# titoeb/RecModel

Measured on AMD Instinct MI355X. Metric: ALS user+item row-updates/sec, higher is better.
Workload: dtype f32; 1 GPU; cfg3: WMF k=128+bias, 10000000x1000000 CSR, 99990947 nnz, alpha-log confidence, gamma=0.1, zipf_a=0.0; n_items=1000000, nnz=99990947, k=128, bias=True

## Files before the change

recmodel_amd/csrc/wmf_dense.hip:

```cpp
#include "wmf_common.h"
#include "wmf_internal.h"

#include <utility>

template <int NFB, int NSPLIT, int S>
__device__ __forceinline__ void gram_body(const float* __restrict__ Y, int64_t m, int f, int ld, int bias,
                                          float* __restrict__ partial, int64_t step_lo, int64_t step_hi) {
    constexpr int NT = NFB * (NFB + 1) / 2;
    constexpr int NACC = (NT + NSPLIT - 1) / NSPLIT;
    const int lane = threadIdx.x & 63;
    const int r = lane & 15, q = lane >> 4;
    f32x4 acc[NACC];
#pragma unroll
    for (int i = 0; i < NACC; ++i) acc[i] = f32x4{0.f, 0.f, 0.f, 0.f};

    constexpr int U = 4;
    float cur[U][NFB], nxt[U][NFB];
    const int last_col = min(16 * (NFB - 1) + r, ld - 1);
    const float col_mask_last = (16 * (NFB - 1) + r < f) ? 1.f : 0.f;
    auto load_trip = [&](int64_t s0, float (&fr)[U][NFB]) {
#pragma unroll
        for (int uu = 0; uu < U; ++uu) {
            const int64_t row = min(4 * (s0 + uu) + q, m - 1);
            const float* yrow = Y + row * (int64_t)ld;
#pragma unroll
            for (int fb = 0; fb < NFB - 1; ++fb) fr[uu][fb] = yrow[16 * fb + r];
            fr[uu][NFB - 1] = yrow[last_col];
        }
    };
    if (step_lo < step_hi) load_trip(step_lo, cur);
    for (int64_t s0 = step_lo; s0 < step_hi; s0 += U) {
        if (s0 + U < step_hi) load_trip(s0 + U, nxt);
#pragma unroll
        for (int uu = 0; uu < U; ++uu) {
            const int64_t s = s0 + uu;
            const float rmask = (s < step_hi && 4 * s + q < m) ? 1.f : 0.f;
            float frag[NFB];
#pragma unroll
            for (int fb = 0; fb < NFB; ++fb) frag[fb] = cur[uu][fb] * rmask;
            frag[NFB - 1] *= col_mask_last;
            if (bias && r == 0) frag[0] = rmask;
            int t = 0;
#pragma unroll
            for (int bi = 0; bi < NFB; ++bi) {
#pragma unroll
                for (int bj = bi; bj < NFB; ++bj, ++t) {
                    if (t % NSPLIT == S) acc[t / NSPLIT] = WMF_MFMA16(frag[bi], frag[bj], acc[t / NSPLIT]);
                }
            }
        }
#pragma unroll
        for (int uu = 0; uu < U; ++uu)
#pragma unroll
            for (int fb = 0; fb < NFB; ++fb) cur[uu][fb] = nxt[uu][fb];
    }
    float* out = partial + (int64_t)blockIdx.x * NT * 256;
    int t = 0;
#pragma unroll
    for (int bi = 0; bi < NFB; ++bi) {
#pragma unroll
        for (int bj = bi; bj < NFB; ++bj, ++t) {
            if (t % NSPLIT == S) {
#pragma unroll
                for (int reg = 0; reg < 4; ++reg) out[(t * 4 + reg) * 64 + lane] = acc[t / NSPLIT][reg];
            }
        }
    }
}

typedef __bf16 gram_bf16x8 __attribute__((ext_vector_type(8)));
template <int NFB>
__device__ __forceinline__ void gram_body6(const float* __restrict__ Y, int64_t m, int f, int ld, int bias,
                                           float* __restrict__ partial, int64_t step_lo, int64_t step_hi) {
    constexpr int NT = NFB * (NFB + 1) / 2;
    const int lane = threadIdx.x;
    const int r = lane & 15, q = lane >> 4;
    f32x4 acc[NT];
#pragma unroll
    for (int i = 0; i < NT; ++i) acc[i] = f32x4{0.f, 0.f, 0.f, 0.f};
    const int last_col = min(16 * (NFB - 1) + r, ld - 1);
    const float col_mask_last = (16 * (NFB - 1) + r < f) ? 1.f : 0.f;
    const int64_t row_lo = 32 * step_lo, row_hi = m, stride = 32 * step_hi;
    float cur[8][NFB], nxt[8][NFB];
    auto load_chunk = [&](int64_t c0, float (&fr)[8][NFB]) {
#pragma unroll
        for (int j = 0; j < 8; ++j) {
            const int64_t row = min(c0 + 8 * q + j, m - 1);
            const float* yrow = Y + row * (int64_t)ld;
#pragma unroll
            for (int fb = 0; fb < NFB - 1; ++fb) fr[j][fb] = yrow[16 * fb + r];
            fr[j][NFB - 1] = yrow[last_col];
        }
    };
    if (row_lo < row_hi) load_chunk(row_lo, cur);
    for (int64_t c0 = row_lo; c0 < row_hi; c0 += stride) {
        if (c0 + stride < row_hi) load_chunk(c0 + stride, nxt);
        gram_bf16x8 hi[NFB], mid[NFB], lo[NFB];
#pragma unroll
        for (int j = 0; j < 8; ++j) {
            const float rmask = (c0 + 8 * q + j < row_hi) ? 1.f : 0.f;
#pragma unroll
            for (int fb = 0; fb < NFB; ++fb) {
                float x = cur[j][fb] * rmask;
                if (fb == NFB - 1) x *= col_mask_last;
                if (fb == 0 && bias && r == 0) x = rmask;
                const __bf16 h = (__bf16)x;
                const float r1 = x - (float)h;
                const __bf16 md = (__bf16)r1;
                hi[fb][j] = h; mid[fb][j] = md; lo[fb][j] = (__bf16)(r1 - (float)md);
            }
        }
        int t0 = 0;
#pragma unroll
        for (int bi = 0; bi < NFB; ++bi) {
#pragma unroll
            for (int bj = bi; bj < NFB; ++bj) acc[t0 + bj - bi] = __builtin_amdgcn_mfma_f32_16x16x32_bf16(lo[bi], hi[bj], acc[t0 + bj - bi], 0, 0, 0);
#pragma unroll
            for (int bj = bi; bj < NFB; ++bj) acc[t0 + bj - bi] = __builtin_amdgcn_mfma_f32_16x16x32_bf16(mid[bi], mid[bj], acc[t0 + bj - bi], 0, 0, 0);
#pragma unroll
            for (int bj = bi; bj < NFB; ++bj) acc[t0 + bj - bi] = __builtin_amdgcn_mfma_f32_16x16x32_bf16(hi[bi], lo[bj], acc[t0 + bj - bi], 0, 0, 0);
#pragma unroll
            for (int bj = bi; bj < NFB; ++bj) acc[t0 + bj - bi] = __builtin_amdgcn_mfma_f32_16x16x32_bf16(mid[bi], hi[bj], acc[t0 + bj - bi], 0, 0, 0);
#pragma unroll
            for (int bj = bi; bj < NFB; ++bj) acc[t0 + bj - bi] = __builtin_amdgcn_mfma_f32_16x16x32_bf16(hi[bi], mid[bj], acc[t0 + bj - bi], 0, 0, 0);
#pragma unroll
            for (int bj = bi; bj < NFB; ++bj) acc[t0 + bj - bi] = __builtin_amdgcn_mfma_f32_16x16x32_bf16(hi[bi], hi[bj], acc[t0 + bj - bi], 0, 0, 0);
            t0 += NFB - bi;
        }
#pragma unroll
        for (int j = 0; j < 8; ++j)
#pragma unroll
            for (int fb = 0; fb < NFB; ++fb) cur[j][fb] = nxt[j][fb];
    }
    float* out = partial + (int64_t)blockIdx.x * NT * 256;
#pragma unroll
    for (int t = 0; t < NT; ++t)
#pragma unroll
        for (int reg = 0; reg < 4; ++reg) out[(t * 4 + reg) * 64 + lane] = acc[t][reg];
}

template <int NFB>
__global__ __launch_bounds__(64) void gram6_kernel(const float* __restrict__ Y, int64_t m, int f, int ld, int bias,
                                                   float* __restrict__ partial, int64_t steps_per_wave) {
    gram_body6<NFB>(Y, m, f, ld, bias, partial, blockIdx.x, gridDim.x);
}

template <int NFB, int NSPLIT>
__global__ __launch_bounds__(NSPLIT == 1 ? 64 : 256) void gram_kernel(const float* __restrict__ Y, int64_t m, int f, int ld, int bias,
                                                  float* __restrict__ partial, int64_t steps_per_wave) {
    const int64_t nsteps = (m + 3) / 4;
    int64_t lo = (int64_t)blockIdx.x * steps_per_wave;
    int64_t hi = lo + steps_per_wave;
    if (hi > nsteps) hi = nsteps;
    if (lo > hi) lo = hi;
    if constexpr (NSPLIT == 1) {
        gram_body<NFB, 1, 0>(Y, m, f, ld, bias, partial, lo, hi);
    } else {
        switch (__builtin_amdgcn_readfirstlane(threadIdx.x >> 6)) {
            case 0: gram_body<NFB, NSPLIT, 0>(Y, m, f, ld, bias, partial, lo, hi); break;
            case 1: gram_body<NFB, NSPLIT, 1>(Y, m, f, ld, bias, partial, lo, hi); break;
            case 2: gram_body<NFB, NSPLIT, 2>(Y, m, f, ld, bias, partial, lo, hi); break;
            default: gram_body<NFB, NSPLIT, 3>(Y, m, f, ld, bias, partial, lo, hi); break;
        }
    }
}

#define WMF_GRAM_SLICES 32
__global__ __launch_bounds__(256) void gram_reduce1_kernel(const float* __restrict__ partial, int nwaves, int f, int nfb,
                                                           double* __restrict__ slices) {
    const int e = blockIdx.x * blockDim.x + threadIdx.x;
    if (e >= f * f) return;
    int i = e / f, j = e % f;
    if (i > j) { int tmp = i; i = j; j = tmp; }
    const int bi = i >> 4, bj = j >> 4, ri = i & 15, cj = j & 15;
    const int t = bi * nfb - (bi * (bi - 1)) / 2 + (bj - bi);
    const int lane = cj + 16 * (ri >> 2), reg = ri & 3;
    const int nt = nfb * (nfb + 1) / 2;
    const float* p = partial + ((int64_t)t * 4 + reg) * 64 + lane;
    const int per = (nwaves + WMF_GRAM_SLICES - 1) / WMF_GRAM_SLICES;
    const int w0 = blockIdx.y * per, w1 = min(nwaves, w0 + per);
    double s = 0.0;
    for (int w = w0; w < w1; ++w) s += (double)p[(int64_t)w * nt * 256];
    slices[(int64_t)blockIdx.y * f * f + e] = s;
}

__global__ __launch_bounds__(256) void gram_reduce2_kernel(const double* __restrict__ slices, int f, double* __restrict__ G) {
    const int e = blockIdx.x * blockDim.x + threadIdx.x;
    if (e >= f * f) return;
    double s = 0.0;
#pragma unroll 8
    for (int k = 0; k < WMF_GRAM_SLICES; ++k) s += slices[(int64_t)k * f * f + e];
    G[e] = s;
}

template <int NFB>
static int launch_gram_nfb(const float* Y, int64_t m, int f, int ld, int bias, float* partial, int nwaves,
                           hipStream_t st) {
    const int64_t nsteps = (m + 3) / 4;
    const int64_t spw = (nsteps + nwaves - 1) / nwaves;
    if constexpr (NFB >= 7 && NFB <= 9) {
        if (!(wmf_debug_flags & WMF_DBG_F32_GRAM)) {
            static const char* nm = wmf_kname("gram6_kernel<%d>", NFB);
            WMF_LAUNCH(nm, (gram6_kernel<NFB>), dim3(nwaves), dim3(64), 0, st, Y, m, f, ld, bias, partial, spw);
            return 0;
        }
    }
    if constexpr (NFB <= 9) {
        static const char* nm = wmf_kname("gram_kernel<%d, 1>", NFB);
        WMF_LAUNCH(nm, (gram_kernel<NFB, 1>), dim3(nwaves), dim3(64), 0, st, Y, m, f, ld, bias, partial, spw);
    } else {
        static const char* nm = wmf_kname("gram_kernel<%d, 4>", NFB);
        WMF_LAUNCH(nm, (gram_kernel<NFB, 4>), dim3(nwaves), dim3(256), 0, st, Y, m, f, ld, bias, partial, spw);
    }
    return 0;
}

int wmf_gram_max_waves(int f) {
    const int64_t nfb = (f + 15) / 16, nt = nfb * (nfb + 1) / 2;
    int64_t cap = ((int64_t)64 << 20) / (nt * 1024);
    if (cap > WMF_GRAM_MAX_WAVES) cap = WMF_GRAM_MAX_WAVES;
    return (int)(cap < 64 ? 64 : cap);
}

int wmf_gram_nwaves(int64_t m, int f) {
    int64_t nsteps = (m + 3) / 4;
    int64_t want = (nsteps + 31) / 32;
    if (want < 1) want = 1;
    const int cap = wmf_gram_max_waves(f);
    if (want > cap) want = cap;
    if (want > 1024) want -= want % 1024;
    return (int)want;
}

int wmf_launch_gram(const float* Y, int64_t m, int f, int ld, int bias, double* G_sum, float* partial, double* slices,
                    hipStream_t st) {
    if (m <= 0) return hipMemsetAsync(G_sum, 0, (size_t)f * f * sizeof(double), st) == hipSuccess ? 0 : -1;
    const int nfb = (f + 15) / 16;
    const int nwaves = wmf_gram_nwaves(m, f);
    switch (nfb) {
#define C(N) case N: launch_gram_nfb<N>(Y, m, f, ld, bias, partial, nwaves, st); break;
        C(1) C(2) C(3) C(4) C(5) C(6) C(7) C(8) C(9) C(10) C(11) C(12) C(13) C(14) C(15) C(16) C(17)
#undef C
        default: return -1;
    }
    WMF_LAUNCH("gram_reduce1_kernel", gram_reduce1_kernel, dim3((f * f + 255) / 256, WMF_GRAM_SLICES), dim3(256), 0, st, partial,
               nwaves, f, nfb, slices);
    WMF_LAUNCH("gram_reduce2_kernel", gram_reduce2_kernel, dim3((f * f + 255) / 256), dim3(256), 0, st, slices, f, G_sum);
    return 0;
}

__device__ __forceinline__ double rl_f64(double v, int lane) {
    const int lo = __builtin_amdgcn_readlane(__double2loint(v), lane);
    const int hi = __builtin_amdgcn_readlane(__double2hiint(v), lane);
    return __hiloint2double(hi, lo);
}

typedef double f64x4 __attribute__((ext_vector_type(4)));
#define WMF_MFMA16_F64(a, b, c) __builtin_amdgcn_mfma_f64_16x16x4f64((a), (b), (c), 0, 0, 0)
constexpr int FZ_LD = 66;

__device__ __forceinline__ f64x4 fz_mul_abt(const double* A, int la, const double* B, int lb, f64x4 c, int r, int q, double sign) {
#pragma unroll
    for (int kk = 0; kk < 4; ++kk) c = WMF_MFMA16_F64(sign * A[r * la + 4 * kk + q], B[r * lb + 4 * kk + q], c);
    return c;
}
__device__ __forceinline__ f64x4 fz_mul_ab(const double* A, int la, const double* B, int lb, f64x4 c, int r, int q, double sign) {
#pragma unroll
    for (int kk = 0; kk < 4; ++kk) c = WMF_MFMA16_F64(sign * A[r * la + 4 * kk + q], B[(4 * kk + q) * lb + r], c);
    return c;
}
__device__ __forceinline__ f64x4 fz_load(const double* T, int lt, int r, int q) {
    return f64x4{T[q * lt + r], T[(q + 4) * lt + r], T[(q + 8) * lt + r], T[(q + 12) * lt + r]};
}
__device__ __forceinline__ void fz_store(double* T, int lt, const f64x4& c, int r, int q) {
#pragma unroll
    for (int v = 0; v < 4; ++v) T[(q + 4 * v) * lt + r] = c[v];
}
__device__ __noinline__ int fz_diag(const double* D, double* Lt, double* Xt, int lt, int lane) {
    const int row = lane & 15;
    double a[16];
#pragma unroll
    for (int j = 0; j < 16; ++j) a[j] = D[row * lt + j];
    int fail = 0;
    double rinv[16];
#pragma unroll
    for (int K = 0; K < 16; ++K) {
        const double dk = rl_f64(a[K], K);
        if (!(dk > 0.0) && !fail) fail = K + 1;
        double y = __builtin_amdgcn_rsq(dk);
        y = y * (1.5 - 0.5 * dk * y * y);
        y = y * (1.5 - 0.5 * dk * y * y);
        rinv[K] = y;
        a[K] *= y;
#pragma unroll
        for (int j = K + 1; j < 16; ++j) a[j] -= a[K] * rl_f64(a[K], j);
    }
    double x[16];
#pragma unroll
    for (int i = 0; i < 16; ++i) {
        double sacc = (i == row) ? 1.0 : 0.0;
#pragma unroll
        for (int k = 0; k < i; ++k) sacc -= rl_f64(a[k], i) * x[k];
        x[i] = sacc * rinv[i];
    }
    if (lane < 16) {
#pragma unroll
        for (int j = 0; j < 16; ++j) {
            Lt[row * lt + j] = (j <= row) ? a[j] : 0.0;
            Xt[j * lt + row] = x[j];
        }
    }
    return fail;
}

__global__ __launch_bounds__(64, 1) void factorize64m_kernel(const double* __restrict__ G, int f, int ld, double lambda,
                                                             float* __restrict__ Wwhite, float* __restrict__ Wunwhite,
                                                             int32_t* __restrict__ info) {
    __shared__ __attribute__((aligned(16))) double Gs[64 * FZ_LD];
    __shared__ __attribute__((aligned(16))) double Xs[64 * FZ_LD];
    __shared__ __attribute__((aligned(16))) double Ts[16 * FZ_LD];
    const int lane = threadIdx.x, r = lane & 15, q = lane >> 4;
    const int nb = (f + 15) >> 4;
#pragma unroll 16
    for (int i = 0; i < 64; ++i) {
        const int j = lane;
        double v = (i == j) ? 1.0 : 0.0;
        const double gv = G[min(i, f - 1) * f + min(j, f - 1)];
        if (i < f && j < f) v = gv + (i == j ? lambda : 0.0);
        Gs[i * FZ_LD + j] = v;
        Xs[i * FZ_LD + j] = 0.0;
    }
    __builtin_amdgcn_fence(__ATOMIC_RELEASE, "wavefront");
    __builtin_amdgcn_wave_barrier();
    int fail = 0;
    auto tile = [&](double* M, int bi, int bj) { return M + (16 * bi) * FZ_LD + 16 * bj; };
    auto sync = [&]() { __builtin_amdgcn_fence(__ATOMIC_RELEASE, "wavefront"); __builtin_amdgcn_wave_barrier(); };
    for (int p = 0; p < nb; ++p) {
        const int bad = fz_diag(tile(Gs, p, p), tile(Gs, p, p), tile(Xs, p, p), FZ_LD, lane);
        if (bad && !fail) fail = 16 * p + bad;
        sync();
        for (int i = p + 1; i < nb; ++i) {
            const f64x4 c = fz_mul_abt(tile(Gs, i, p), FZ_LD, tile(Xs, p, p), FZ_LD, f64x4{0.0, 0.0, 0.0, 0.0}, r, q, 1.0);
            sync();
            fz_store(tile(Gs, i, p), FZ_LD, c, r, q);
            sync();
        }
        for (int i = p + 1; i < nb; ++i)
            for (int j = p + 1; j <= i; ++j) {
                const f64x4 c = fz_mul_abt(tile(Gs, i, p), FZ_LD, tile(Gs, j, p), FZ_LD, fz_load(tile(Gs, i, j), FZ_LD, r, q), r, q, -1.0);
                fz_store(tile(Gs, i, j), FZ_LD, c, r, q);
            }
        sync();
    }
    for (int p = 0; p < nb; ++p)
        for (int i = p + 1; i < nb; ++i) {
            f64x4 sacc = f64x4{0.0, 0.0, 0.0, 0.0};
            for (int k = p; k < i; ++k) sacc = fz_mul_ab(tile(Gs, i, k), FZ_LD, tile(Xs, k, p), FZ_LD, sacc, r, q, 1.0);
            fz_store(Ts, FZ_LD, sacc, r, q);
            sync();
            const f64x4 c = fz_mul_ab(tile(Xs, i, i), FZ_LD, Ts, FZ_LD, f64x4{0.0, 0.0, 0.0, 0.0}, r, q, -1.0);
            fz_store(tile(Xs, i, p), FZ_LD, c, r, q);
            sync();
        }
    const bool ok = fail == 0;
    if (lane == 0 && !ok) *info = fail;
#pragma unroll 8
    for (int i = 0; i < 64; ++i) {
        if (i >= f) break;
        for (int j = lane; j < ld; j += 64) {
            float wu = 0.f, ww = 0.f;
            if (j < f && ok) { wu = (float)Xs[i * FZ_LD + j]; ww = (float)Xs[j * FZ_LD + i]; }
            Wunwhite[i * ld + j] = wu;
            Wwhite[i * ld + j] = ww;
        }
    }
}

__global__ __launch_bounds__(512, 1) void factorize_blocked_kernel(const double* __restrict__ G, int f, int ld, double lambda,
                                                                   float* __restrict__ Wwhite, float* __restrict__ Wunwhite,
                                                                   int32_t* __restrict__ info, double* __restrict__ work) {
    __shared__ __attribute__((aligned(16))) double Ts[8][16 * 18];
    __shared__ int bad;
    const int tid = threadIdx.x, lane = tid & 63, r = lane & 15, q = lane >> 4;
    const int wave = __builtin_amdgcn_readfirstlane(tid >> 6);
    const int nb = (f + 15) >> 4, fp = 16 * nb, LD = fp + 2;
    double* A = work;
    double* X = work + (size_t)fp * LD;
    if (tid == 0) bad = 0;
    for (int e = tid; e < fp * fp; e += 512) {
        const int i = e / fp, j = e % fp;
        double v = (i == j) ? 1.0 : 0.0;
        if (i < f && j < f) v = G[i * f + j] + (i == j ? lambda : 0.0);
        A[i * LD + j] = v;
        X[i * LD + j] = 0.0;
    }
    __syncthreads();
    auto tile = [&](double* M, int bi, int bj) { return M + (size_t)(16 * bi) * LD + 16 * bj; };
    for (int p = 0; p < nb; ++p) {
        if (wave == 0) {
            const int fail = fz_diag(tile(A, p, p), tile(A, p, p), tile(X, p, p), LD, lane);
            if (fail && lane == 0 && !bad) bad = 16 * p + fail;
        }
        __syncthreads();
        for (int i = p + 1 + wave; i < nb; i += 8) {
            const f64x4 c = fz_mul_abt(tile(A, i, p), LD, tile(X, p, p), LD, f64x4{0.0, 0.0, 0.0, 0.0}, r, q, 1.0);
            fz_store(tile(A, i, p), LD, c, r, q);
        }
        __syncthreads();
        int t = 0;
        for (int i = p + 1; i < nb; ++i)
            for (int j = p + 1; j <= i; ++j, ++t) {
                if ((t & 7) != wave) continue;
                const f64x4 c = fz_mul_abt(tile(A, i, p), LD, tile(A, j, p), LD, fz_load(tile(A, i, j), LD, r, q), r, q, -1.0);
                fz_store(tile(A, i, j), LD, c, r, q);
            }
        __syncthreads();
    }
    double* ts = Ts[wave];
    for (int p = wave; p < nb; p += 8)
        for (int i = p + 1; i < nb; ++i) {
            f64x4 sacc = f64x4{0.0, 0.0, 0.0, 0.0};
            for (int k = p; k < i; ++k) sacc = fz_mul_ab(tile(A, i, k), LD, tile(X, k, p), LD, sacc, r, q, 1.0);
            fz_store(ts, 18, sacc, r, q);
            __builtin_amdgcn_fence(__ATOMIC_RELEASE, "wavefront");
            __builtin_amdgcn_wave_barrier();
            const f64x4 c = fz_mul_ab(tile(X, i, i), LD, ts, 18, f64x4{0.0, 0.0, 0.0, 0.0}, r, q, -1.0);
            fz_store(tile(X, i, p), LD, c, r, q);
            __builtin_amdgcn_fence(__ATOMIC_RELEASE, "wavefront");
            __builtin_amdgcn_wave_barrier();
        }
    __syncthreads();
    const bool ok = bad == 0;
    if (tid == 0 && !ok) *info = bad;
    for (int e = tid; e < f * ld; e += 512) {
        const int i = e / ld, j = e % ld;
        float wu = 0.f, ww = 0.f;
        if (j < f && ok) { wu = (float)X[i * LD + j]; ww = (float)X[j * LD + i]; }
        Wunwhite[e] = wu;
        Wwhite[e] = ww;
    }
}

int wmf_launch_factorize(const double* G_sum, int f, int ld, double lambda, float* Wwhite, float* Wunwhite,
                         int32_t* info, double* gA, hipStream_t st) {
    if (f <= 64) {
        WmfProfScope ps("factorize64m_kernel", st);
        hipLaunchKernelGGL(factorize64m_kernel, dim3(1), dim3(64), 0, st, G_sum, f, ld, lambda, Wwhite, Wunwhite, info);
        return 0;
    }
    WmfProfScope ps("factorize_blocked_kernel", st);
    hipLaunchKernelGGL(factorize_blocked_kernel, dim3(1), dim3(512), 0, st, G_sum, f, ld, lambda, Wwhite, Wunwhite, info, gA);
    return 0;
}

template <int NFB, bool W_IN_LDS, int NB0 = 0, int NBW = NFB>
__global__ __launch_bounds__(512) void transform_kernel(const float* __restrict__ in, int64_t m, int f, int ld,
                                                        const float* __restrict__ W, int set_col0_one,
                                                        float* __restrict__ out, float* __restrict__ col0_out,
                                                        int64_t nblocks16) {
    extern __shared__ __attribute__((aligned(16))) char smem_raw[];
    float* Wl = reinterpret_cast<float*>(smem_raw);
    constexpr int KP = 16 * NFB;
    constexpr int NP = 16 * NBW;
    constexpr int LDW = NP + 4;
    const int tid = threadIdx.x;
    __shared__ int nz[NFB * NBW];
    for (int e = tid; e < NFB * NBW; e += 512) nz[e] = 0;
    __syncthreads();
    for (int e = tid; e < KP * LDW; e += 512) {
        const int a = e / LDW, b = e % LDW, col = 16 * NB0 + b;
        const float v = (a < f && b < NP && col < f) ? W[a * ld + col] : 0.f;
        if constexpr (W_IN_LDS) Wl[e] = v;
        if (v != 0.f) nz[(a >> 4) * NBW + (b >> 4)] = 1;
    }
    __syncthreads();
    const int lane = tid & 63, wv = tid >> 6;
    const int r = lane & 15, q = lane >> 4;
    const int nch = ld >> 2;
    unsigned tmask[NFB];
#pragma unroll
    for (int t = 0; t < NFB; ++t) {
        unsigned mk = 0;
#pragma unroll
        for (int nb = 0; nb < NBW; ++nb) mk |= nz[t * NBW + nb] ? (1u << nb) : 0u;
        tmask[t] = __builtin_amdgcn_readfirstlane(mk);
    }
    constexpr bool DBL = NFB <= 11;
    const int64_t stride = (int64_t)gridDim.x * 8;
    auto request = [&](int64_t blk, float4 (&x)[NFB]) {
        const int64_t row = blk * 16 + r;
        const float4* irow = reinterpret_cast<const float4*>(in + (row < m ? row : 0) * (int64_t)ld);
#pragma unroll
        for (int t = 0; t < NFB; ++t) x[t] = irow[min(4 * t + q, nch - 1)];
    };
    auto block = [&](int64_t blk, float4 (&xc)[NFB], float4 (&xn)[NFB]) {
        if constexpr (DBL) { if (blk + stride < nblocks16) request(blk + stride, xn); }
        const int64_t row = blk * 16 + r;
        const bool rok = row < m;
        f32x4 acc[NBW];
#pragma unroll
        for (int nb = 0; nb < NBW; ++nb) acc[nb] = f32x4{0.f, 0.f, 0.f, 0.f};
#pragma unroll
        for (int t = 0; t < NFB; ++t) {
            const int c = 4 * t + q;
            const int k0 = 4 * c;
            float xe[4] = {xc[t].x, xc[t].y, xc[t].z, xc[t].w};
            if (t == NFB - 1) {
#pragma unroll
                for (int e = 0; e < 4; ++e) if (!(c < nch && k0 + e < f)) xe[e] = 0.f;
            }
            if (t == 0 && set_col0_one && q == 0) {
                if (rok && col0_out && NB0 == 0) col0_out[set_col0_one == 2 ? 2 * row + 1 : row] = xe[0];
                xe[0] = 1.f;
            }
            unsigned mv = tmask[t];
            asm volatile("" : "+v"(mv));
            const unsigned mk = __builtin_amdgcn_readfirstlane(mv);
#pragma unroll
            for (int nb = 0; nb < NBW; ++nb) {
                if (!(mk & (1u << nb))) continue;
#pragma unroll
                for (int e = 0; e < 4; ++e) {
                    const int k = k0 + e;
                    float b;
                    if constexpr (W_IN_LDS) {
                        b = Wl[k * LDW + 16 * nb + r];
                    } else {
                        const int col = 16 * (NB0 + nb) + r;
                        b = (k < f && col < f) ? W[k * ld + col] : 0.f;
                    }
                    acc[nb] = WMF_MFMA16(xe[e], b, acc[nb]);
                }
            }
        }
#pragma unroll
        for (int reg = 0; reg < 4; ++reg) {
            const int64_t orow = blk * 16 + 4 * q + reg;
            if (orow < m) {
                const bool sp = set_col0_one == 2;
                const int wid = sp ? f - 1 : ld;
                float* o = out + orow * (int64_t)wid;
#pragma unroll
                for (int nb = 0; nb < NBW; ++nb) {
                    const int col = 16 * (NB0 + nb) + r;
                    if (col < wid) o[col] = acc[nb][reg];
                    else if (sp && col == f - 1) col0_out[2 * orow] = acc[nb][reg];
                }
            }
        }
    };
    int64_t blk = (int64_t)blockIdx.x * 8 + wv;
    if constexpr (DBL) {
        float4 xa[NFB], xb[NFB];
        if (blk < nblocks16) request(blk, xa);
        while (blk < nblocks16) {
            block(blk, xa, xb);
            blk += stride;
            if (blk >= nblocks16) break;
            block(blk, xb, xa);
            blk += stride;
        }
    } else {
        float4 xa[NFB];
        for (; blk < nblocks16; blk += stride) {
            request(blk, xa);
            block(blk, xa, xa);
        }
    }
}

template <int NFB>
__global__ __launch_bounds__(512) void transform6_kernel(const float* __restrict__ in, int64_t m, int f, int ld,
                                                         const float* __restrict__ W, int set_col0_one,
                                                         float* __restrict__ out, float* __restrict__ col0_out,
                                                         int64_t nblocks16) {
    extern __shared__ __attribute__((aligned(16))) char smem_raw[];
    constexpr int NP = 16 * NFB;
    constexpr int NKC = (NP + 31) / 32;
    constexpr int KS = 176;
    static_assert(32 * NKC <= KS, "K does not fit the LDS row");
    __bf16* Wt = reinterpret_cast<__bf16*>(smem_raw);
    __shared__ int nz[NKC * NFB];
    const int tid = threadIdx.x;
    for (int e = tid; e < NKC * NFB; e += 512) nz[e] = 0;
    __syncthreads();
    const bool roll_n = set_col0_one == 3, roll_k = set_col0_one == 4;
    for (int e = tid; e < NP * KS; e += 512) {
        const int n = e / KS, k = e % KS;
        const int ns = (roll_n && n < f) ? (n + 1 == f ? 0 : n + 1) : n, ks = (roll_k && k < f) ? (k + 1 == f ? 0 : k + 1) : k;
        const float v = (k < f && n < f) ? W[ks * ld + ns] : 0.f;
        const __bf16 h = (__bf16)v;
        const float r1 = v - (float)h;
        const __bf16 md = (__bf16)r1;
        Wt[e] = h;
        Wt[NP * KS + e] = md;
        Wt[2 * NP * KS + e] = (__bf16)(r1 - (float)md);
        if (v != 0.f) nz[(k >> 5) * NFB + (n >> 4)] = 1;
    }
    __syncthreads();
    const int lane = tid & 63, wv = tid >> 6;
    const int r = lane & 15, q = lane >> 4;
    const int nch = ld >> 2;
    unsigned cmask[NKC];
#pragma unroll
    for (int c = 0; c < NKC; ++c) {
        unsigned mk = 0;
#pragma unroll
        for (int nb = 0; nb < NFB; ++nb) mk |= nz[c * NFB + nb] ? (1u << nb) : 0u;
        cmask[c] = __builtin_amdgcn_readfirstlane(mk);
    }
    typedef __bf16 bf16x8_t __attribute__((ext_vector_type(8)));
    const bf16x8_t* Wl = reinterpret_cast<const bf16x8_t*>(Wt);
    const int64_t stride = (int64_t)gridDim.x * 8;
    auto request = [&](int64_t blk, float4 (&x)[2 * NKC]) {
        const int64_t row = blk * 16 + r;
        const float4* irow = reinterpret_cast<const float4*>(in + (row < m ? row : 0) * (int64_t)ld);
#pragma unroll
        for (int c = 0; c < NKC; ++c) {
            x[2 * c] = irow[min(8 * c + 2 * q, nch - 1)];
            x[2 * c + 1] = irow[min(8 * c + 2 * q + 1, nch - 1)];
        }
    };
    const bool in_one = set_col0_one >= 1 && set_col0_one <= 3;
    const bool sp = set_col0_one == 2 || set_col0_one == 3;
    auto block = [&](int64_t blk, float4 (&xc)[2 * NKC]) {
        const int64_t row = blk * 16 + r;
        const bool rok = row < m;
        float bias_of_row = 0.f;
        f32x4 acc[NFB];
#pragma unroll
        for (int nb = 0; nb < NFB; ++nb) acc[nb] = f32x4{0.f, 0.f, 0.f, 0.f};
#pragma unroll
        for (int c = 0; c < NKC; ++c) {
            const int k0 = 32 * c + 8 * q;
            float xe[8] = {xc[2 * c].x, xc[2 * c].y, xc[2 * c].z, xc[2 * c].w, xc[2 * c + 1].x, xc[2 * c + 1].y, xc[2 * c + 1].z, xc[2 * c + 1].w};
            if (32 * c + 32 > f) {
#pragma unroll
                for (int e = 0; e < 8; ++e) if (!(k0 + e < f)) xe[e] = 0.f;
            }
            if (c == 0 && in_one && q == 0) {
                if (rok && col0_out) col0_out[sp ? 2 * row + 1 : row] = xe[0];
                bias_of_row = xe[0];
                xe[0] = 1.f;
            }
            bf16x8_t ah, am, al;
#pragma unroll
            for (int e = 0; e < 8; ++e) {
                const __bf16 h = (__bf16)xe[e];
                const float r1 = xe[e] - (float)h;
                const __bf16 md = (__bf16)r1;
                ah[e] = h; am[e] = md; al[e] = (__bf16)(r1 - (float)md);
            }
            unsigned mv = cmask[c];
            asm volatile("" : "+v"(mv));
            const unsigned mk = __builtin_amdgcn_readfirstlane(mv);
#pragma unroll
            for (int nb = 0; nb < NFB; ++nb) {
                if (!(mk & (1u << nb))) continue;
                const int at = ((16 * nb + r) * KS + 32 * c + 8 * q) / 8;
                const bf16x8_t bh = Wl[at], bm = Wl[NP * KS / 8 + at], bl = Wl[2 * NP * KS / 8 + at];
                f32x4 cc = acc[nb];
                cc = __builtin_amdgcn_mfma_f32_16x16x32_bf16(al, bh, cc, 0, 0, 0);
                cc = __builtin_amdgcn_mfma_f32_16x16x32_bf16(am, bm, cc, 0, 0, 0);
                cc = __builtin_amdgcn_mfma_f32_16x16x32_bf16(ah, bl, cc, 0, 0, 0);
                cc = __builtin_amdgcn_mfma_f32_16x16x32_bf16(am, bh, cc, 0, 0, 0);
                cc = __builtin_amdgcn_mfma_f32_16x16x32_bf16(ah, bm, cc, 0, 0, 0);
                cc = __builtin_amdgcn_mfma_f32_16x16x32_bf16(ah, bh, cc, 0, 0, 0);
                acc[nb] = cc;
            }
        }
#pragma unroll
        for (int reg = 0; reg < 4; ++reg) {
            const int64_t orow = blk * 16 + 4 * q + reg;
            const unsigned bbits = set_col0_one == 3 ? (unsigned)__builtin_amdgcn_ds_bpermute((4 * q + reg) * 4, __builtin_bit_cast(int, bias_of_row)) : 0u;
            if (orow < m) {
                const int wid = sp ? f - 1 : ld;
                float* o = out + orow * (int64_t)wid;
#pragma unroll
                for (int nb = 0; nb < NFB; ++nb) {
                    const int col = 16 * nb + r;
                    float v = acc[nb][reg];
                    if (set_col0_one == 3 && col < 128 && (col & 7) < 2)
                        v = __builtin_bit_cast(float, (__builtin_bit_cast(unsigned, v) & ~1u) | ((bbits >> (2 * (col >> 3) + (col & 7))) & 1u));
                    if (col < wid) o[col] = v;
                    else if (sp && col == f - 1) col0_out[2 * orow] = v;
                }
            }
        }
    };
    float4 xa[2 * NKC];
    for (int64_t blk = (int64_t)blockIdx.x * 8 + wv; blk < nblocks16; blk += stride) {
        request(blk, xa);
        block(blk, xa);
    }
}

template <int NFB>
static void launch_transform6(const float* in, int64_t m, int f, int ld, const float* W, int set_col0_one, float* out,
                              float* col0_out, int64_t grid, int64_t nblk, hipStream_t st) {
    constexpr size_t lds = (size_t)3 * 16 * NFB * 176 * 2;
    static_assert(lds <= 158 * 1024, "W planes do not fit LDS");
    static bool attr_set = false;
    if (!attr_set) {
        (void)hipFuncSetAttribute((const void*)transform6_kernel<NFB>, hipFuncAttributeMaxDynamicSharedMemorySize, (int)lds);
        attr_set = true;
    }
    static const char* nm = wmf_kname("transform6_kernel<%d>", NFB);
    WMF_LAUNCH(nm, (transform6_kernel<NFB>), dim3((unsigned)grid), dim3(512), lds, st, in, m, f, ld, W, set_col0_one, out,
               col0_out, nblk);
}

template <int NFB, int NB0, int NBW>
static void launch_transform_slice(const float* in, int64_t m, int f, int ld, const float* W, int set_col0_one, float* out,
                                   float* col0_out, int64_t grid, int64_t nblk, hipStream_t st) {
    constexpr size_t lds = (size_t)16 * NFB * (16 * NBW + 4) * 4;
    static_assert(lds <= 150 * 1024, "slice too wide");
    static bool attr_set = false;
    if (!attr_set) {
        (void)hipFuncSetAttribute((const void*)transform_kernel<NFB, true, NB0, NBW>, hipFuncAttributeMaxDynamicSharedMemorySize,
                                  (int)lds);
        attr_set = true;
    }
    static const char* nm = wmf_kname("transform_kernel<%d, true, %d, %d>", NFB, NB0, NBW);
    WMF_LAUNCH(nm, (transform_kernel<NFB, true, NB0, NBW>), dim3((unsigned)grid), dim3(512), lds, st, in, m, f, ld, W,
               set_col0_one, out, col0_out, nblk);
}

template <int NFB>
static void launch_transform_nfb(const float* in, int64_t m, int f, int ld, const float* W, int set_col0_one, float* out,
                                 float* col0_out, hipStream_t st) {
    constexpr int KP = 16 * NFB, LDW = KP + 4;
    constexpr size_t lds = (size_t)KP * LDW * 4;
    const int64_t nblk = (m + 15) / 16;
    int64_t grid = (nblk + 7) / 8;
    if (grid > 1024) grid = 1024;
    if (grid < 1) grid = 1;
    constexpr bool WIDE = NFB >= 7 && NFB <= 9;
    if constexpr (WIDE) {
        if (!WMF_LAB_BUILD || !(wmf_debug_flags & WMF_DBG_F32_TRANSFORM)) {
            launch_transform6<NFB>(in, m, f, ld, W, set_col0_one, out, col0_out, grid, nblk, st);
            return;
        }
    }
    if constexpr (WIDE && !WMF_LAB_BUILD) {
    } else if constexpr (lds <= 150 * 1024) {
        launch_transform_slice<NFB, 0, NFB>(in, m, f, ld, W, set_col0_one, out, col0_out, grid, nblk, st);
    } else if (in != out) {
        constexpr int H = (NFB + 1) / 2;
        if constexpr (H <= 8) {
            launch_transform_slice<NFB, 0, H>(in, m, f, ld, W, set_col0_one, out, col0_out, grid, nblk, st);
            launch_transform_slice<NFB, H, NFB - H>(in, m, f, ld, W, set_col0_one, out, col0_out, grid, nblk, st);
        } else {
            launch_transform_slice<NFB, 0, 6>(in, m, f, ld, W, set_col0_one, out, col0_out, grid, nblk, st);
            launch_transform_slice<NFB, 6, 6>(in, m, f, ld, W, set_col0_one, out, col0_out, grid, nblk, st);
            launch_transform_slice<NFB, 12, NFB - 12>(in, m, f, ld, W, set_col0_one, out, col0_out, grid, nblk, st);
        }
    } else {
        static const char* nm = wmf_kname("transform_kernel<%d, false, 0, %d>", NFB, NFB);
        WMF_LAUNCH(nm, (transform_kernel<NFB, false>), dim3((unsigned)grid), dim3(512), 0, st, in, m, f, ld, W,
                   set_col0_one, out, col0_out, nblk);
    }
}

int wmf_launch_transform(const float* in, int64_t m, int f, int ld, const float* W, int set_col0_one, float* out,
                         float* col0_out, hipStream_t st) {
    if (m <= 0) return 0;
    const int nfb = (f + 15) / 16;
    if (set_col0_one == 3 || set_col0_one == 4) {
        if (!wmf_rolled_layout(f, ld)) return -1;
    } else {
        set_col0_one = set_col0_one ? (wmf_split_layout(f, ld) ? 2 : 1) : 0;
    }
    if ((set_col0_one == 2 || set_col0_one == 3) && (!col0_out || in == out)) return -3;
    switch (nfb) {
#define C(N) case N: launch_transform_nfb<N>(in, m, f, ld, W, set_col0_one, out, col0_out, st); break;
        C(1) C(2) C(3) C(4) C(5) C(6) C(7) C(8) C(9) C(10) C(11) C(12) C(13) C(14) C(15) C(16) C(17)
#undef C
        default: return -1;
    }
    return 0;
}
```

Measured before the change: 409.5 million row-updates/s.

## Software-pipeline gram loads with MFMA and specialize transform tile patterns at compile time

The gram kernel now streams loads and bf16 splitting one column block at a time, interleaved with the MFMA chain of the previous block. sched_group_barrier hints interleave VALU, MFMA and VMEM work, replacing the old whole-chunk prefetch and register copy. The triangular-solve transform kernel gains compile-time specialisations for known upper/lower (optionally rolled) nonzero tile patterns, which unroll the tile list and double-buffer the LDS fetches of W. It falls back to the generic path when the runtime mask does not match. The bias-bit insertion is also hoisted out of the store loop. These changes increase code size and register pressure and depend on the compiler honouring the scheduling hints.

```diff
diff --git a/recmodel_amd/csrc/wmf_dense.hip b/recmodel_amd/csrc/wmf_dense.hip
--- a/recmodel_amd/csrc/wmf_dense.hip
+++ b/recmodel_amd/csrc/wmf_dense.hip
@@ -1,7 +1,16 @@
 #include "wmf_common.h"
 #include "wmf_internal.h"
+#include "wmf_dense_patterns.h"
 
 #include <utility>
+
+template <int I0, int N, class F>
+__device__ __forceinline__ void wmf_static_for(F&& f) {
+    if constexpr (I0 < N) {
+        f(std::integral_constant<int, I0>{});
+        wmf_static_for<I0 + 1, N>(f);
+    }
+}
 
 template <int NFB, int NSPLIT, int S>
 __device__ __forceinline__ void gram_body(const float* __restrict__ Y, int64_t m, int f, int ld, int bias,
@@ -81,38 +90,55 @@
     const int last_col = min(16 * (NFB - 1) + r, ld - 1);
     const float col_mask_last = (16 * (NFB - 1) + r < f) ? 1.f : 0.f;
     const int64_t row_lo = 32 * step_lo, row_hi = m, stride = 32 * step_hi;
-    float cur[8][NFB], nxt[8][NFB];
-    auto load_chunk = [&](int64_t c0, float (&fr)[8][NFB]) {
+    float raw[8][NFB];
+    gram_bf16x8 hi[NFB], mid[NFB], lo[NFB];
+    int64_t ro[8];
+    float rmask[8];
+    auto set_rows = [&](int64_t c0) {
+#pragma unroll
+        for (int j = 0; j < 8; ++j) ro[j] = min(c0 + 8 * q + j, m - 1) * (int64_t)ld;
+    };
+    auto set_masks = [&](int64_t c0) {
+#pragma unroll
+        for (int j = 0; j < 8; ++j) rmask[j] = (c0 + 8 * q + j < row_hi) ? 1.f : 0.f;
+    };
+    auto load_col = [&](int fb) {
+#pragma unroll
+        for (int j = 0; j < 8; ++j) raw[j][fb] = Y[ro[j] + (fb < NFB - 1 ? 16 * fb + r : last_col)];
+    };
+    auto split_col = [&](int fb) {
 #pragma unroll
         for (int j = 0; j < 8; ++j) {
-            const int64_t row = min(c0 + 8 * q + j, m - 1);
-            const float* yrow = Y + row * (int64_t)ld;
-#pragma unroll
-            for (int fb = 0; fb < NFB - 1; ++fb) fr[j][fb] = yrow[16 * fb + r];
-            fr[j][NFB - 1] = yrow[last_col];
-        }
-    };
-    if (row_lo < row_hi) load_chunk(row_lo, cur);
+            float x = raw[j][fb] * rmask[j];
+            if (fb == NFB - 1) x *= col_mask_last;
+            if (fb == 0 && bias && r == 0) x = rmask[j];
+            asm volatile("" : "+v"(x));
+            const __bf16 h = (__bf16)x;
+            const float r1 = x - (float)h;
+            const __bf16 md = (__bf16)r1;
+            hi[fb][j] = h; mid[fb][j] = md; lo[fb][j] = (__bf16)(r1 - (float)md);
+        }
+        asm volatile("" : "+v"(hi[fb]), "+v"(mid[fb]), "+v"(lo[fb]));
+    };
+    set_rows(row_lo);
+    set_masks(row_lo);
+#pragma unroll
+    for (int fb = 0; fb < NFB; ++fb) load_col(fb);
+    set_rows(row_lo + stride);
+#pragma unroll
+    for (int fb = 0; fb < NFB; ++fb) { split_col(fb); load_col(fb); }
     for (int64_t c0 = row_lo; c0 < row_hi; c0 += stride) {
-        if (c0 + stride < row_hi) load_chunk(c0 + stride, nxt);
-        gram_bf16x8 hi[NFB], mid[NFB], lo[NFB];
-#pragma unroll
-        for (int j = 0; j < 8; ++j) {
-            const float rmask = (c0 + 8 * q + j < row_hi) ? 1.f : 0.f;
-#pragma unroll
-            for (int fb = 0; fb < NFB; ++fb) {
-                float x = cur[j][fb] * rmask;
-                if (fb == NFB - 1) x *= col_mask_last;
-                if (fb == 0 && bias && r == 0) x = rmask;
-                const __bf16 h = (__bf16)x;
-                const float r1 = x - (float)h;
-                const __bf16 md = (__bf16)r1;
-                hi[fb][j] = h; mid[fb][j] = md; lo[fb][j] = (__bf16)(r1 - (float)md);
-            }
-        }
-        int t0 = 0;
-#pragma unroll
-        for (int bi = 0; bi < NFB; ++bi) {
+        wmf_static_for<0, NFB>([&](auto bi_c) {
+            constexpr int bi = decltype(bi_c)::value, t0 = bi * NFB - bi * (bi - 1) / 2;
+            if constexpr (bi == 0) {
+                set_masks(c0 + stride);
+                set_rows(c0 + 2 * stride);
+#pragma unroll
+                for (int j = 0; j < 8; ++j) asm volatile("" : "+v"(ro[j]), "+v"(rmask[j]));
+            } else {
+                split_col(bi - 1);
+                load_col(bi - 1);
+            }
 #pragma unroll
             for (int bj = bi; bj < NFB; ++bj) acc[t0 + bj - bi] = __builtin_amdgcn_mfma_f32_16x16x32_bf16(lo[bi], hi[bj], acc[t0 + bj - bi], 0, 0, 0);
 #pragma unroll
@@ -125,12 +151,20 @@
             for (int bj = bi; bj < NFB; ++bj) acc[t0 + bj - bi] = __builtin_amdgcn_mfma_f32_16x16x32_bf16(hi[bi], mid[bj], acc[t0 + bj - bi], 0, 0, 0);
 #pragma unroll
             for (int bj = bi; bj < NFB; ++bj) acc[t0 + bj - bi] = __builtin_amdgcn_mfma_f32_16x16x32_bf16(hi[bi], hi[bj], acc[t0 + bj - bi], 0, 0, 0);
-            t0 += NFB - bi;
-        }
-#pragma unroll
-        for (int j = 0; j < 8; ++j)
-#pragma unroll
-            for (int fb = 0; fb < NFB; ++fb) cur[j][fb] = nxt[j][fb];
+            {
+                constexpr int SPLIT_VALU = 96;
+                constexpr int nm = 6 * (NFB - bi), per = bi == 0 ? 3 : (SPLIT_VALU + nm - 1) / nm;
+#pragma unroll
+                for (int i = 0; i < nm; ++i) {
+                    __builtin_amdgcn_sched_group_barrier(0x008, 1, 0);
+                    __builtin_amdgcn_sched_group_barrier(0x002, per, 0);
+                    __builtin_amdgcn_sched_group_barrier(0x020, 1, 0);
+                }
+            }
+            __builtin_amdgcn_sched_barrier(0);
+        });
+        split_col(NFB - 1);
+        load_col(NFB - 1);
     }
     float* out = partial + (int64_t)blockIdx.x * NT * 256;
 #pragma unroll
@@ -568,6 +602,24 @@
         }
     }
 }
+
+template <int NFB, int PAT>
+struct wmf_t6_tiles {
+    static constexpr int NKC = (16 * NFB + 31) / 32;
+    struct table { unsigned mask[NKC]; int index[NKC][NFB]; int c[NKC * NFB + 1], nb[NKC * NFB + 1]; int count; };
+    static constexpr table make() {
+        table t{};
+        for (int c = 0; c < NKC; ++c) {
+            t.mask[c] = wmf_t6_pattern_mask(NFB, PAT, c);
+            for (int nb = 0; nb < NFB; ++nb) {
+                t.index[c][nb] = -1;
+                if (t.mask[c] >> nb & 1) { t.index[c][nb] = t.count; t.c[t.count] = c; t.nb[t.count] = nb; ++t.count; }
+            }
+        }
+        return t;
+    }
+    static constexpr table T = make();
+};
 
 template <int NFB>
 __global__ __launch_bounds__(512) void transform6_kernel(const float* __restrict__ in, int64_t m, int f, int ld,
@@ -623,13 +675,66 @@
     };
     const bool in_one = set_col0_one >= 1 && set_col0_one <= 3;
     const bool sp = set_col0_one == 2 || set_col0_one == 3;
-    auto block = [&](int64_t blk, float4 (&xc)[2 * NKC]) {
+    const bf16x8_t* wb = Wl + r * (KS / 8) + q;
+    auto block = [&](int64_t blk, float4 (&xc)[2 * NKC], auto pat_c) {
+        constexpr int PAT = decltype(pat_c)::value;
         const int64_t row = blk * 16 + r;
         const bool rok = row < m;
         float bias_of_row = 0.f;
         f32x4 acc[NFB];
 #pragma unroll
         for (int nb = 0; nb < NFB; ++nb) acc[nb] = f32x4{0.f, 0.f, 0.f, 0.f};
+        if constexpr (PAT != WMF_T6_GENERIC) {
+            using TL = wmf_t6_tiles<NFB, PAT>;
+            static_assert(TL::T.mask[0] != 0, "chunk 0 takes the bias out of the input");
+            bf16x8_t b[2][3];
+            auto fetch = [&](int t, bf16x8_t (&bb)[3]) {
+                const int at = 16 * TL::T.nb[t] * (KS / 8) + 4 * TL::T.c[t];
+                bb[0] = wb[at]; bb[1] = wb[NP * KS / 8 + at]; bb[2] = wb[2 * NP * KS / 8 + at];
+            };
+            fetch(0, b[0]);
+            wmf_static_for<0, NKC>([&](auto c_c) {
+                constexpr int c = decltype(c_c)::value;
+                if constexpr (TL::T.mask[c] != 0) {
+                    const int k0 = 32 * c + 8 * q;
+                    float xe[8] = {xc[2 * c].x, xc[2 * c].y, xc[2 * c].z, xc[2 * c].w, xc[2 * c + 1].x, xc[2 * c + 1].y, xc[2 * c + 1].z, xc[2 * c + 1].w};
+                    if constexpr (32 * c + 32 > 16 * (NFB - 1) + 1) {
+#pragma unroll
+                        for (int e = 0; e < 8; ++e) xe[e] = k0 + e < f ? xe[e] : 0.f;
+                    }
+                    if (c == 0 && in_one && q == 0) {
+                        if (rok && col0_out) col0_out[sp ? 2 * row + 1 : row] = xe[0];
+                        bias_of_row = xe[0];
+                        xe[0] = 1.f;
+                    }
+                    bf16x8_t ah, am, al;
+#pragma unroll
+                    for (int e = 0; e < 8; ++e) {
+                        const __bf16 h = (__bf16)xe[e];
+                        const float r1 = xe[e] - (float)h;
+                        const __bf16 md = (__bf16)r1;
+                        ah[e] = h; am[e] = md; al[e] = (__bf16)(r1 - (float)md);
+                    }
+                    wmf_static_for<0, NFB>([&](auto nb_c) {
+                        constexpr int nb = decltype(nb_c)::value, t = TL::T.index[c][nb];
+                        if constexpr (t >= 0) {
+                            if constexpr (t + 1 < TL::T.count) fetch(t + 1, b[(t + 1) & 1]);
+                            const bf16x8_t bh = b[t & 1][0], bm = b[t & 1][1], bl = b[t & 1][2];
+                            f32x4 cc = acc[nb];
+                            cc = __builtin_amdgcn_mfma_f32_16x16x32_bf16(al, bh, cc, 0, 0, 0);
+                            cc = __builtin_amdgcn_mfma_f32_16x16x32_bf16(am, bm, cc, 0, 0, 0);
+                            cc = __builtin_amdgcn_mfma_f32_16x16x32_bf16(ah, bl, cc, 0, 0, 0);
+                            cc = __builtin_amdgcn_mfma_f32_16x16x32_bf16(am, bh, cc, 0, 0, 0);
+                            cc = __builtin_amdgcn_mfma_f32_16x16x32_bf16(ah, bm, cc, 0, 0, 0);
+                            cc = __builtin_amdgcn_mfma_f32_16x16x32_bf16(ah, bh, cc, 0, 0, 0);
+                            acc[nb] = cc;
+                            __builtin_amdgcn_sched_group_barrier(0x100, 3, 0);
+                            __builtin_amdgcn_sched_group_barrier(0x008, 6, 0);
+                        }
+                    });
+                }
+            });
+        } else {
 #pragma unroll
         for (int c = 0; c < NKC; ++c) {
             const int k0 = 32 * c + 8 * q;
@@ -669,30 +774,55 @@
                 acc[nb] = cc;
             }
         }
+        }
+        if (set_col0_one == 3) {
+            const bool ins = (r & 7) < 2;
+            const int sh0 = 2 * (r >> 3) + (r & 7);
+#pragma unroll
+            for (int reg = 0; reg < 4; ++reg) {
+                const unsigned bbits = (unsigned)__builtin_amdgcn_ds_bpermute((4 * q + reg) * 4, __builtin_bit_cast(int, bias_of_row));
+#pragma unroll
+                for (int nb = 0; nb < NFB && nb < 8; ++nb) {
+                    const float v = acc[nb][reg];
+                    const unsigned vb = __builtin_bit_cast(unsigned, v);
+                    acc[nb][reg] = __builtin_bit_cast(float, ins ? (vb & ~1u) | ((bbits >> (4 * nb + sh0)) & 1u) : vb);
+                }
+            }
+        }
 #pragma unroll
         for (int reg = 0; reg < 4; ++reg) {
             const int64_t orow = blk * 16 + 4 * q + reg;
-            const unsigned bbits = set_col0_one == 3 ? (unsigned)__builtin_amdgcn_ds_bpermute((4 * q + reg) * 4, __builtin_bit_cast(int, bias_of_row)) : 0u;
             if (orow < m) {
                 const int wid = sp ? f - 1 : ld;
                 float* o = out + orow * (int64_t)wid;
 #pragma unroll
                 for (int nb = 0; nb < NFB; ++nb) {
                     const int col = 16 * nb + r;
-                    float v = acc[nb][reg];
-                    if (set_col0_one == 3 && col < 128 && (col & 7) < 2)
-                        v = __builtin_bit_cast(float, (__builtin_bit_cast(unsigned, v) & ~1u) | ((bbits >> (2 * (col >> 3) + (col & 7))) & 1u));
-                    if (col < wid) o[col] = v;
-                    else if (sp && col == f - 1) col0_out[2 * orow] = v;
+                    if (nb < NFB - 1 || col < wid) o[col] = acc[nb][reg];
+                    else if (sp && col == f - 1) col0_out[2 * orow] = acc[nb][reg];
                 }
             }
         }
     };
-    float4 xa[2 * NKC];
-    for (int64_t blk = (int64_t)blockIdx.x * 8 + wv; blk < nblocks16; blk += stride) {
-        request(blk, xa);
-        block(blk, xa);
-    }
+    auto run = [&](auto pat_c) {
+        float4 xa[2 * NKC];
+        for (int64_t blk = (int64_t)blockIdx.x * 8 + wv; blk < nblocks16; blk += stride) {
+            request(blk, xa);
+            block(blk, xa, pat_c);
+        }
+    };
+    auto fits = [&](auto pat_c) {
+        bool ok = true;
+#pragma unroll
+        for (int c = 0; c < NKC; ++c) ok = ok && (cmask[c] & ~wmf_t6_tiles<NFB, decltype(pat_c)::value>::T.mask[c]) == 0;
+        return ok;
+    };
+    using std::integral_constant;
+    if (fits(integral_constant<int, WMF_T6_UPPER>{})) run(integral_constant<int, WMF_T6_UPPER>{});
+    else if (fits(integral_constant<int, WMF_T6_UPPER_ROLLED>{})) run(integral_constant<int, WMF_T6_UPPER_ROLLED>{});
+    else if (fits(integral_constant<int, WMF_T6_LOWER_ROLLED>{})) run(integral_constant<int, WMF_T6_LOWER_ROLLED>{});
+    else if (fits(integral_constant<int, WMF_T6_LOWER>{})) run(integral_constant<int, WMF_T6_LOWER>{});
+    else run(integral_constant<int, WMF_T6_GENERIC>{});
 }
 
 template <int NFB>
diff --git a/recmodel_amd/csrc/wmf_dense_patterns.h b/recmodel_amd/csrc/wmf_dense_patterns.h
--- /dev/null
+++ b/recmodel_amd/csrc/wmf_dense_patterns.h
@@ -0,0 +1,25 @@
+#pragma once
+
+enum wmf_t6_pattern {
+    WMF_T6_GENERIC = -1,
+    WMF_T6_UPPER = 0,
+    WMF_T6_UPPER_ROLLED = 1,
+    WMF_T6_LOWER_ROLLED = 2,
+    WMF_T6_LOWER = 3,
+    WMF_T6_NPATTERNS = 4
+};
+
+constexpr unsigned wmf_t6_pattern_mask(int nfb, int pattern, int c) {
+    const bool roll_n = pattern == WMF_T6_UPPER_ROLLED, roll_k = pattern == WMF_T6_LOWER_ROLLED;
+    const bool upper = pattern == WMF_T6_UPPER || pattern == WMF_T6_UPPER_ROLLED;
+    const int f = (roll_n || roll_k) ? 16 * (nfb - 1) + 1 : 16 * nfb;
+    unsigned mk = 0;
+    for (int k = 32 * c; k < 32 * c + 32 && k < f; ++k) {
+        const int ks = roll_k ? (k + 1 == f ? 0 : k + 1) : k;
+        for (int n = 0; n < f; ++n) {
+            const int ns = roll_n ? (n + 1 == f ? 0 : n + 1) : n;
+            if (upper ? ks <= ns : ks >= ns) mk |= 1u << (n >> 4);
+        }
+    }
+    return mk;
+}
```

New measurement: 409.8 million row-updates/s, median of 3. No clear change (+0.1%).
